# vgl-hub/teloscope

Measured on AMD Instinct MI355X. Metric: Gbases/s scanned (whole node), 3 Gb FASTA TTAGGG w=1000 s=500, higher is better.
Workload: dtype u8; 1 GPU; configs[1]: synthetic 3.00 Gb / 200 contigs, -c TTAGGG -p TTAGGG,TCAGGG,TGAGGG,TTGGGG -x 1 -w 1000 -s 500 -r -g -e -m -i, 124 patterns k=6; bases=3000000000, windows=6000095, matches=91510666, tiles=260970

## Files before the change

teloscope_amd/csrc/capi.cpp:

```cpp
#include <hip/hip_runtime.h>
#include <immintrin.h>

#include <algorithm>
#include <atomic>
#include <thread>
#include <cstdio>
#include <cstddef>
#include <cstdlib>
#include <chrono>
#include <cstring>
#include <limits>
#include <memory>
#include <mutex>
#include <string>
#include <tuple>
#include <vector>

#include <cctype>
#include <pthread.h>
#include <sched.h>
#include <sys/mman.h>

#include "capi_internal.hpp"

// ... 713 lines not shown
    if (!ctx) return TS_ERR_INVALID_ARG;
    DEVICE_TRY(ctx);
    int ok = 0;
    if (ts_k_streams_concurrent(stream_a, stream_b, &ok) != 0) return ctx->fail(TS_ERR_HIP, "stream probe failed");
    return ok;
}

int ts_refresh_env(ts_ctx *ctx) {
    if (!ctx) return TS_ERR_INVALID_ARG;
    std::lock_guard<std::mutex> lk(ctx->api_mtx);
    read_env_knobs(ctx);
    return TS_OK;
}

int ts_takes_text_input(const ts_ctx *ctx, int tips_only) {
    std::string why;
    return ctx && ((tips_only ? ctx->fast_ok : ts_full_scan_supported(ctx, why)) || ctx->generic_ok) ? 1 : 0;
}

int ts_device_input_stats(const ts_ctx *ctx, uint64_t out[4]) {
    if (!ctx || !out) return TS_ERR_INVALID_ARG;
    for (int i = 0; i < 4; ++i) out[i] = ctx->device_input_stats[i].load(std::memory_order_relaxed);
    return TS_OK;
}

int ts_upload_stats(const ts_ctx *ctx, uint64_t out[8]) {
    if (!ctx || !out) return TS_ERR_INVALID_ARG;
    for (int i = 0; i < 8; ++i) out[i] = ctx->upload_stats[i].load(std::memory_order_relaxed);
    return TS_OK;
}

ts_batch *ts_batch_create(ts_ctx *ctx, const uint64_t *seg_lens, const uint64_t *abs_pos,
                          size_t n_segs, int tips_only, uint64_t match_capacity) {
    if (!ctx) return nullptr;
    if (n_segs && !seg_lens) { ctx->fail(TS_ERR_INVALID_ARG, "ts_batch_create: null seg_lens"); return nullptr; }
    std::string why;
    if (tips_only ? !ctx->fast_ok : !ts_full_scan_supported(ctx, why)) {
        ctx->fail(TS_ERR_UNSUPPORTED, "unsupported parameter set: " + (tips_only ? ctx->why_not : why));
        return nullptr;
    }

    ts_batch *b = new ts_batch();
    b->ctx = ctx;
    b->tips = tips_only != 0;
    uint32_t wpt = 1;
    if (!plan_geometry(ctx, b->tips, b->kp, wpt, why)) {
        ctx->fail(TS_ERR_UNSUPPORTED, "unsupported parameter set: " + why);
        delete b;
        return nullptr;
    }
    b->wpt = wpt;
    if (getenv("TS_TIMING"))
        fprintf(stderr, "ts_batch_create: %s scan, k=%u (%s pair table), %u x %u waves per CU, %u chunks and %u windows per tile, LDS %d B per workgroup "
                        "(match queue %u, record stage %u, %u accumulator copies)\n", b->tips ? "tips-only" : "window", ctx->k,
                ctx->pair_byte_table ? "byte" : "2-bit",
                b->kp.wgs_per_cu, b->kp.waves_per_wg, b->kp.nch, wpt, ts_k_lds_bytes(&b->kp), (unsigned)TS_LIST, b->kp.stage_cap, b->kp.acc_copies);
    const uint64_t tile_bases = (uint64_t)wpt * b->kp.s;
    const uint32_t tl = ctx->params.terminal_limit;

    uint64_t off = 0, wins = 0;
    b->segs.resize(n_segs);
    for (size_t i = 0; i < n_segs; ++i) {
        SegPlan &sp = b->segs[i];
        sp.len = seg_lens[i];
        sp.abs_pos = abs_pos ? abs_pos[i] : 0;
        sp.in_off = off;
        off += (sp.len + 15) & ~15ull;
        sp.first_tile = (uint32_t)b->tiles.size();
        if (b->tips) {
            const uint32_t twice = 2u * tl;
            if (sp.len > twice) {
                add_region_tiles(b, sp, (uint32_t)i, 0, tl, tile_bases, 1, false);
                add_region_tiles(b, sp, (uint32_t)i, sp.len - tl, tl, tile_bases, 1, false);
            } else if (sp.len > 0) {
                add_region_tiles(b, sp, (uint32_t)i, 0, sp.len, tile_bases, 1, false);
            }
        } else {
            sp.win_base = wins;
            sp.n_windows = ceil_div(sp.len, ctx->params.step);
            wins += sp.n_windows;
            if (sp.len > 0) add_region_tiles(b, sp, (uint32_t)i, 0, sp.len, tile_bases, wpt, true);
        }
        sp.n_tiles = (uint32_t)b->tiles.size() - sp.first_tile;
        b->total_bases += sp.len;
    }
    b->input_bytes = off + TS_IN_PAD;
    b->n_windows = wins;
    b->match_cap_request = match_capacity;
    if (b->tiles.size() >= 0x7FFFFFFFull) {
        ctx->fail(TS_ERR_UNSUPPORTED, "too many tiles in one batch");
        delete b;
        return nullptr;
    }
    b->lds_bytes = (uint32_t)ts_k_lds_bytes(&b->kp);
    b->kp.rec16 = (b->kp.stage_u16 && ctx->knobs.rec16) ? 1u : 0u;
    set_range(b, 0, b->tiles.size());
    return b;
}

void ts_batch_destroy(ts_batch *b) {
    if (!b) return;
    ts_ctx *c = b->ctx;
    if (c->device != kNoDevice) {
        DeviceGuard g(c->device);
        for (DevBuf *d : {&b->d_in, &b->d_tiles, &b->d_windows, &b->d_matches, &b->d_tile_off, &b->d_stats, &b->d_fill, &b->d_tickets,
                          &b->d_segtab, &b->d_dense, &b->d_dense_base, &b->d_scan_tmp, &b->d_readtab, &b->d_shard_segs,
                          &b->d_shard_bounds, &b->d_shard_tmp, &b->d_shard_cand, &b->d_vis, &b->d_chain, &b->d_zone})
            c->pool.give(std::move(*d));
        for (hipEvent_t e : b->evs)
// ... 806 lines not shown
```

teloscope_amd/csrc/kernels.hip:

```cpp
#include <hip/hip_runtime.h>
#include <stdint.h>

#include <type_traits>

#include "ts_device.h"
#include "ts_internal.h"

#define set_prio(p) __builtin_amdgcn_s_setprio(p)
constexpr int kPrioPass = 3;
constexpr int kPrioAppend = 2;
constexpr int kPrioWindows = 2;

namespace {

typedef unsigned long long u64;
#define LDS __attribute__((address_space(3)))
typedef uint32_t u32x2 __attribute__((ext_vector_type(2)));
typedef LDS unsigned char lds_u8;
typedef LDS uint16_t lds_u16;
typedef LDS uint32_t lds_u32;

__device__ __forceinline__ lds_u16 *lds_at16(uint32_t addr) { return (lds_u16 *)(uintptr_t)addr; }
__device__ __forceinline__ lds_u8 *lds_at8(uint32_t addr) { return (lds_u8 *)(uintptr_t)addr; }

__host__ __device__ inline uint32_t align16(uint32_t x) { return (x + 15u) & ~15u; }

struct SliceLayout { uint32_t codes, rec, wacc, stage, park, bytes; };

__host__ __device__ inline SliceLayout slice_layout(const TsScanParams &P) {
    SliceLayout s;
    uint32_t o = 0;
    s.codes = o; o += align16((P.nch * 63u + 1u) * 8u);
    s.rec = o; o += (P.windows_on && P.nuc_on) ? align16((P.max_windows + P.halo_blocks) * 16u) : 0u;
    s.wacc = o; o += P.windows_on ? align16((P.max_windows + (P.acc_blocks ? P.halo_blocks : 0u)) * 8u * (P.acc_copies + (P.acc_blocks ? 1u : 0u))) : 0u;
    s.stage = o; o += (P.stage_cap + 64u) * (P.stage_u16 ? 2u : 4u);
    s.park = o; o += 32u;
    s.bytes = o;
    return s;
}

__host__ __device__ inline uint32_t queue_region(const TsScanParams &P) {
    const uint32_t a = TS_LIST * 2u;
    return (P.table_rows * 4u + P.fc_bytes + a - 1u) & ~(a - 1u);
}

__host__ __device__ inline uint32_t lds_total(const TsScanParams &P) {
    return queue_region(P) + P.waves_per_wg * (TS_LIST * 2u + slice_layout(P).bytes);
}

template <bool FC_BYTES, bool PAIR_BYTES, int WAVES_EU, bool EMIT, bool FAST>
__global__ __launch_bounds__(TS_MAX_WG_THREADS, WAVES_EU)
void ts_scan_tiles(const TsScanParams P) {
    const bool st16 = FAST ? true : P.stage_u16 != 0u;
    const bool accb = FAST ? true : P.acc_blocks != 0u;
    extern __shared__ __attribute__((aligned(16))) unsigned char lds_raw[];
    const uint32_t tid = threadIdx.x;
    const uint32_t lane = tid & 63u;
    const uint32_t wave = (uint32_t)__builtin_amdgcn_readfirstlane((int)(tid >> 6));

    const uint32_t table_bytes = P.table_rows * 4u + P.fc_bytes;
    {
        const uint4 *src = (const uint4 *)P.table;
        uint4 *dst = (uint4 *)lds_raw;
        const uint32_t n16 = table_bytes >> 4;
        for (uint32_t i = tid; i < n16; i += blockDim.x) dst[i] = src[i];
    }
    __syncthreads();

    const SliceLayout SL = slice_layout(P);
    lds_u8 *lds = (lds_u8 *)lds_raw;
    uint32_t qbase = queue_region(P) + wave * (TS_LIST * 2u);
    uint32_t qmask = TS_LIST * 2u - 2u;
    asm volatile("" : "+v"(qbase));
    asm volatile("" : "+s"(qmask));
    lds_u8 *slice = lds + queue_region(P) + P.waves_per_wg * (TS_LIST * 2u) + wave * SL.bytes;
    lds_u32 *codes = (lds_u32 *)(slice + SL.codes);
    lds_u32 *rec = (lds_u32 *)(slice + SL.rec);
    lds_u32 *stage = (lds_u32 *)(slice + SL.stage);
    LDS u64 *wacc = (LDS u64 *)(slice + SL.wacc);
    lds_u32 *park = (lds_u32 *)(slice + SL.park);
    const uint32_t acc_rows = P.max_windows + (accb ? P.halo_blocks : 0u);
    const uint32_t acc_off = (lane & (P.acc_copies - 1u)) * acc_rows;

    const uint32_t k = P.k;
    const uint32_t rowbits = 2u * (k + 1u) - 4u;
    const uint32_t kmask = (1u << (2u * k)) - 1u;
    const uint32_t pmask = (1u << (2u * (k + 1u))) - 1u;
    const lds_u32 *fc_table = (const lds_u32 *)(lds + P.table_rows * 4u);
    const lds_u8 *fc_bytes = (const lds_u8 *)fc_table;
    const uint32_t tab_base = (uint32_t)(uintptr_t)lds;
    if (PAIR_BYTES && (tab_base & pmask) != 0u) __builtin_trap();

    const uint32_t total_waves = gridDim.x * P.waves_per_wg;
    const uint32_t gw = blockIdx.x * P.waves_per_wg + wave;
    typedef const TsScanParams __attribute__((address_space(4))) *KernArgs;
    auto tail_params = [&]() -> KernArgs {
        KernArgs q = (KernArgs)__builtin_amdgcn_kernarg_segment_ptr();
        asm volatile("" : "+s"(q));
        return q;
    };
    uint32_t cursor = 0;
    if (EMIT) { park[4] = 0u; park[5] = 0u; }
    const uint32_t nwper = P.halo_blocks + 1u;

    typedef const TsTile __attribute__((address_space(4))) *ConstTiles;
    const ConstTiles const_tiles = (ConstTiles)(uintptr_t)P.tiles;
    uint4 n0 = make_uint4(0, 0, 0, 0), n1 = n0;
// ... 166 lines not shown
                                     "s_and_b64 %[m], %[m], %[canm]\n\t"
                                     "s_bcnt1_i32_b64 %[tmp], %[m]\n\t"
                                     "s_cmp_lg_u64 %[H], 0\n\t"
                                     "s_cselect_b32 %[cc], %[tmp], %[t]"
                                     : [cc] "+s"(ch_cc), [w1] "+s"(ch_w1), [tmp] "=&s"(tmp), [m] "=&s"(m)
                                     : [H] "s"(H), [canm] "s"(canm), [t] "s"(t)
                                     : "scc");
                    }
                }
                ch_last = (uint32_t)__builtin_amdgcn_readlane((int)u, FULL ? 63 : (int)nrow - 1);
            };
            if (!redo) {
                const uint32_t nfull = n & ~63u;
                for (uint32_t i0 = 0; i0 < nfull; i0 += 64u) {
                    const uint32_t o = cursor + base + i0 + ln;
                    const uint32_t r = stage_at(i0 + ln);
                    auto put = [&]() { if (rec16) gstore_lo16(wave_out16 + o, r); else gstore(wave_out + o, r); };
                    if (rec_fit) put();
                    else if (o < cap) put();
                    look(r, 64u, i0, std::true_type{});
                }
                for (uint32_t i0 = nfull; i0 < n; i0 += 64u) {
                    const uint32_t nrow = n - i0 < 64u ? n - i0 : 64u;
                    const uint32_t o = cursor + base + i0 + ln;
                    uint32_t r = 0u;
                    if (ln < nrow) {
                        r = stage_at(i0 + ln);
                        if (o < cap) {
                            if (rec16) gstore_lo16(wave_out16 + o, r);
                            else gstore(wave_out + o, r);
                        }
                    }
                    look(r, nrow, i0, std::false_type{});
                }
            } else {
                for (uint32_t i0 = 0; i0 < n; i0 += 64u) {
                    const uint32_t nrow = n - i0 < 64u ? n - i0 : 64u;
                    const uint32_t o = cursor + base + i0 + ln;
                    uint32_t r = 0u;
                    if (ln < nrow && o < cap)
                        r = rec16 ? (uint32_t)__hip_atomic_load(wave_out16 + o, __ATOMIC_RELAXED, __HIP_MEMORY_SCOPE_AGENT)
                                  : __hip_atomic_load(wave_out + o, __ATOMIC_RELAXED, __HIP_MEMORY_SCOPE_AGENT);
                    look(r, nrow, i0, std::false_type{});
                }
            }
            flushed = done;
            const uint32_t z15 = ch_cc < 0x7FFFu ? ch_cc : 0x7FFFu;
            if (!(ch_w1 & TS_CHAIN_HEADS)) ch_w1 |= z15;
            const u64 voff = vwave + vbase;
            if (ln == 0u) gstore((uint4 *)&Q->tile_chain[4ull * tile], make_uint4((ch_first & 0xFFFFu) | (ch_last << 16), ch_w1 | (z15 << 16), (uint32_t)voff, (uint32_t)(voff >> 32)));
            tile_vis = vout;
            park[4] = vbase + vout;
        };
        if (P.windows_on)
            for (uint32_t it = lane; it < acc_rows * 2u * (P.acc_copies + (accb ? 1u : 0u)); it += 64u) ((lds_u32 *)wacc)[it] = 0u;

        uint32_t qhead = 0, qcount = 0;
        auto drain_queue = [&](const uint32_t threshold) {
            if (qcount >= threshold && qcount > 0u) set_prio(kPrioPass);
            while (qcount >= threshold && qcount > 0u) {
                const uint32_t n = qcount < 64u ? qcount : 64u;
                if (done - flushed + 64u > P.stage_cap) flush_stage();
                const bool live = lane < n;
                const uint32_t xp = live ? (uint32_t)*lds_at16(((qhead + lane * 2u) & qmask) | qbase) : 0u;
                const lds_u32 *cw = codes + __builtin_amdgcn_ubfe(xp, 4, 12);
                const uint32_t kw = __builtin_amdgcn_alignbit(cw[1], cw[0], (xp & 15u) * 2u);
                const uint32_t idx = kw & kmask;
                uint32_t fc;
                if (PAIR_BYTES) fc = __builtin_amdgcn_ubfe((uint32_t)*lds_at8(kw & pmask), 2, 2);
                else if (FC_BYTES) fc = fc_bytes[idx];
                else fc = (fc_table[idx >> 4] >> ((idx & 15u) << 1)) & 3u;
                const uint32_t u = xp - sh;
                uint32_t q = 0u, o = u;
                if (P.windows_on) {
                    uint32_t qs;
                    if (P.div_exact) {
                        q = __umul24(u, P.s_magic22) >> 22; qs = __umul24(q, P.s);
                    } else {
                        q = __umul24(u, P.s_inv) >> 16; qs = __umul24(q, P.s);
                        if (qs > u) { --q; qs -= P.s; }
                    }
                    o = u - qs;
                }
                u64 valid_m = low_bits(n) & ballot64(xp >= sh);
                if (P.straddle_fix) valid_m &= ~ballot64(o + k > P.s);
                const u64 bal = valid_m & ballot64(xp < own_end);
                const bool valid = __builtin_amdgcn_inverse_ballot_w64(valid_m), owned = __builtin_amdgcn_inverse_ballot_w64(bal);
                const uint32_t rank = __builtin_amdgcn_mbcnt_hi((uint32_t)(bal >> 32), __builtin_amdgcn_mbcnt_lo((uint32_t)bal, 0u));
                const uint32_t slot = owned ? (done - flushed) + rank : P.stage_cap + lane;
                const uint32_t record = (u << 2) | fc;
                if (st16) ((lds_u16 *)stage)[slot] = (uint16_t)record; else stage[slot] = record;
                done += (uint32_t)__popcll(bal);
                const u64 can_all = ballot64((fc & 1u) != 0u), fwd_all = ballot64((fc & 2u) != 0u);
                const bool is_can = __builtin_amdgcn_inverse_ballot_w64(can_all), is_fwd = __builtin_amdgcn_inverse_ballot_w64(fwd_all);
                const u64 canm = can_all & bal;
                ccan += (uint32_t)__popcll(canm);
                cfwd += (uint32_t)__popcll(fwd_all & bal);
                const u64 inc = (u64)(is_can ? 1u : 0x10000u) | ((u64)(is_fwd ? 1u : 0x10000u) << 32);
                if (P.windows_on && accb) {
                    if (valid && q < nblk) atomicAdd((unsigned long long *)(wacc + acc_off + q), inc);
                    const u64 over = valid_m & ballot64(o + k > P.s);
                    if (over != 0ull) {
                        if (__builtin_amdgcn_inverse_ballot_w64(over) && q < nblk) atomicAdd((unsigned long long *)(wacc + P.acc_copies * acc_rows + q), inc);
                    }
                } else if (P.windows_on) {
                    for (uint32_t j = 0; j < nwper; ++j) {
                        const uint32_t wi = q - j;
                        const bool in = valid && wi < T.nwin && o + k + j * P.s <= P.w;
                        if (in) atomicAdd((unsigned long long *)(wacc + acc_off + wi), inc);
                    }
                }
                qhead = (qhead + 2u * n) & (TS_LIST * 2u - 1u);
                qcount -= n;
            }
            set_prio(0);
            __builtin_amdgcn_wave_barrier();
        };

        auto scan_chunk = [&](const uint32_t cpos, const uint32_t ch, const uint4 v0, const uint4 v1) -> uint32_t {
            const uint32_t x[8] = {v0.x, v0.y, v0.z, v0.w, v1.x, v1.y, v1.z, v1.w};
            uint32_t t[8], e[8], bad = 0;
#pragma unroll
            for (int i = 0; i < 8; ++i) {
                t[i] = x[i] & 0x06060606u;
                e[i] = __builtin_amdgcn_perm(0xFF47FF54u, 0xFF43FF41u, t[i]);
                bad = __builtin_amdgcn_bitop3_b32(x[i], e[i], bad, 0xBE);
            }
            uint32_t wa = pack16(t), wb = pack16(t + 4);

            const uint32_t pos0 = cpos + lane * 32u;
            uint32_t inv = 0;
            const bool slow = __any((bad & P.fold_mask) != 0u) || (cpos + 2048u > xend);
            if (slow) {
                asm volatile("; non-ACGT bases or segment end in this chunk" ::: "memory");
                uint32_t b4[8];
#pragma unroll
                for (int i = 0; i < 8; ++i) {
                    const uint32_t d = (x[i] & P.fold_mask) ^ e[i];
                    const uint32_t nz = ((((d & 0x7F7F7F7Fu) + 0x7F7F7F7Fu) | d) & 0x80808080u) >> 7;
                    b4[i] = __builtin_amdgcn_udot4(nz, 0x08040201u, 0u, false);
                }
                inv = b4[0] | (b4[1] << 4) | (b4[2] << 8) | (b4[3] << 12) |
                      (b4[4] << 16) | (b4[5] << 20) | (b4[6] << 24) | (b4[7] << 28);
                uint32_t inside = inv;
                if (pos0 < sh) inside &= ~0u << (sh - pos0);
                if (pos0 + 32u > xend) {
                    const uint32_t nv = xend > pos0 ? xend - pos0 : 0u;
                    inside &= ~(~0u << nv);
                    inv |= ~0u << nv;
                }
                if (__any(inside != 0u)) has_invalid = true;
                wa = pack16(t); wb = pack16(t + 4);
            }

            const uint32_t nx = (uint32_t)__builtin_amdgcn_mov_dpp((int)wa, 0x130, 0xf, 0xf, false);

            uint32_t tmp[16], ent[16];
            const uint32_t xa = PAIR_BYTES ? __builtin_amdgcn_alignbit(wb, wa, 16) : 0u;
            const uint32_t xb = PAIR_BYTES ? __builtin_amdgcn_alignbit(nx, wb, 16) : 0u;
#pragma unroll
            for (int j = 0; j < 16; ++j) {
                if (PAIR_BYTES) {
                    tmp[j] = 0;
// ... 45 lines not shown
                    incl = wave_scan_add(nm);
                    total = (uint32_t)__builtin_amdgcn_readlane((int)incl, 63);
                }
                drain_queue(qcount + total > TS_LIST ? 1u : 64u);
                uint32_t o = qhead + 2u * (qcount + incl - nm);
                while (m) {
                    *lds_at16((o & qmask) | qbase) = (uint16_t)(lbase + (uint32_t)__builtin_ctz(m));
                    o += 2u;
                    m &= m - 1u;
                }
                qcount += total;
                __builtin_amdgcn_wave_barrier();
            }
        };
        auto append_pair = [&](const uint32_t mA, const uint32_t cposA, const uint32_t mB, const uint32_t cposB) {
            if (!__any((mA | mB) != 0u)) return;
            set_prio(kPrioAppend);
            const uint32_t nA = __popc(mA), nB = __popc(mB);
            const uint32_t incl = wave_scan_add(nA | (nB << 16));
            const uint32_t tot = (uint32_t)__builtin_amdgcn_readlane((int)incl, 63);
            const uint32_t totA = tot & 0xFFFFu, totB = tot >> 16;
            if (totA + totB + 63u > TS_LIST) {
                asm volatile("; dense pair of chunks" ::: "memory");
                if (totA) append_chunk(mA, cposA, nA, incl & 0xFFFFu, totA);
                if (totB) append_chunk(mB, cposB, nB, incl >> 16, totB);
                set_prio(0);
                return;
            }
            drain_queue(64u);
            set_prio(kPrioAppend);
            uint32_t o = qhead + 2u * (qcount + (incl & 0xFFFFu) - nA), m = mA;
            uint32_t lbase = cposA + lane * 32u;
            while (m) {
                *lds_at16((o & qmask) | qbase) = (uint16_t)(lbase + (uint32_t)__builtin_ctz(m));
                o += 2u;
                m &= m - 1u;
            }
            o = qhead + 2u * (qcount + totA + (incl >> 16) - nB); m = mB;
            lbase = cposB + lane * 32u;
            while (m) {
                *lds_at16((o & qmask) | qbase) = (uint16_t)(lbase + (uint32_t)__builtin_ctz(m));
                o += 2u;
                m &= m - 1u;
            }
            qcount += totA + totB;
            set_prio(0);
            __builtin_amdgcn_wave_barrier();
        };
        {
            const uint32_t last_pos = (uint32_t)__builtin_amdgcn_readfirstlane((int)((nch - 1u) * TS_CHUNK));
            const unsigned char *lsrc = src + lane * 32u;
            uint4 a0 = n0, a1 = n1, b0, b1;
            uint32_t cpos = 0, ch = 0;
            for (uint32_t c = 0; c < nch; c += 2u) {
                const uint32_t p1 = cpos + TS_CHUNK < last_pos ? cpos + TS_CHUNK : last_pos;
                b0 = *(const uint4 *)(lsrc + p1);
                b1 = *(const uint4 *)(lsrc + p1 + 16);
                __builtin_amdgcn_sched_barrier(0);
                const uint32_t mA = scan_chunk(cpos, ch, a0, a1);
                uint32_t mB = 0u;
                const bool pair = c + 1u < nch;
                if (pair) {
                    const uint32_t p2 = cpos + 2u * TS_CHUNK < last_pos ? cpos + 2u * TS_CHUNK : last_pos;
                    a0 = *(const uint4 *)(lsrc + p2);
                    a1 = *(const uint4 *)(lsrc + p2 + 16);
                    __builtin_amdgcn_sched_barrier(0);
                    mB = scan_chunk(cpos + TS_CHUNK, ch + 63u, b0, b1);
                }
                append_pair(mA, cpos, mB, cpos + TS_CHUNK);
                cpos += 2u * TS_CHUNK; ch += 126u;
            }
        }
#define TS_REQUEST_NEXT_TILE()                                                                                                   \
        {                                                                                                                        \
                           \
            __builtin_amdgcn_s_waitcnt(0x0F70);                                                                                  \
            KernArgs Q = tail_params();                                                                                          \
            const bool dyn = Q->dynamic_tiles != 0u;                                                                             \
            tile_next = dyn ? group + Q->ticket_groups * (group_waves + (uint32_t)__builtin_amdgcn_readfirstlane((int)ticket))   \
                            : tile + total_waves;                                                                                \
            if (tile_next < P.ntiles) {                       \
                const unsigned char *ls = P.in + (const_tiles[tile_next].in_off & ~15ull) + lane * 32u;                          \
                n0 = *(const uint4 *)ls; n1 = *(const uint4 *)(ls + 16);                                                         \
                if (dyn && lane == 0) ticket = take_ticket(Q);                         \
            }                                                                                                                    \
        }
        if (!EMIT) TS_REQUEST_NEXT_TILE()
        drain_queue(1u);
        __builtin_amdgcn_wave_barrier();

        set_prio(kPrioWindows);
        if (!EMIT) finish_records();
        if (EMIT) TS_REQUEST_NEXT_TILE()
        if (P.windows_on) {
            auto count_piece = [&](uint32_t xs, uint32_t xe, uint32_t &nL, uint32_t &nH, uint32_t &nG) {
                const uint32_t d0 = xs >> 4, d1 = (xe - 1u) >> 4;
                const uint32_t m0 = ~0u << (2u * (xs & 15u));
                const uint32_t m1 = ~0u >> (2u * (15u - ((xe - 1u) & 15u)));
                auto add2 = [&](uint32_t wA, uint32_t wB) {
                    const uint32_t lo = (wA & 0x55555555u) | ((wB << 1) & 0xAAAAAAAAu);
                    const uint32_t hi = ((wA >> 1) & 0x55555555u) | (wB & 0xAAAAAAAAu);
                    nL += __popc(lo); nH += __popc(hi); nG += __popc(lo & hi);
                };
                uint32_t first = codes[d0] & m0, last = 0u;
                if (d1 == d0) first &= m1; else last = codes[d1] & m1;
                add2(first, last);
                uint32_t d = d0 + 1u;
                for (; d + 2u <= d1; d += 2u) add2(codes[d], codes[d + 1u]);
                if (d < d1) add2(codes[d], 0u);
            };
            auto count_piece_bytes = [&](uint32_t xs, uint32_t xe, uint32_t n[4]) {
                const uint32_t fold = P.fold_mask & 0xFFu;
                for (uint32_t x = xs; x < xe; ++x) {
                    const uint32_t c = (uint32_t)src[x] & fold;
                    n[0] += c == 0x41u; n[1] += c == 0x43u; n[2] += c == 0x47u; n[3] += c == 0x54u;
                }
            };
            const bool by_blocks = P.block_sums != 0u;
            if (P.nuc_on) {
                const uint32_t rows = by_blocks ? T.nwin + P.halo_blocks : T.nwin;
                const uint32_t len = by_blocks ? P.s : P.w;
                for (uint32_t it = lane; it < rows * 4u; it += 64u) rec[it] = 0u;
                uint32_t pshift = 0;
                while (pshift < 2u && (rows << (pshift + 1u)) <= 64u && (len >> (pshift + 1u)) >= 128u) ++pshift;
                const uint32_t piece = (len + (1u << pshift) - 1u) >> pshift;
                __builtin_amdgcn_wave_barrier();
                for (uint32_t it = lane; it < (rows << pshift); it += 64u) {
                    const uint32_t row = it >> pshift, part = it & ((1u << pshift) - 1u);
                    const uint32_t row_end = row * P.s + len < T.nrel ? row * P.s + len : T.nrel;
                    const uint32_t us = row * P.s + part * piece;
                    const uint32_t ue = us + piece < row_end ? us + piece : row_end;
                    if (us >= ue) continue;
                    uint32_t n[4] = {0u, 0u, 0u, 0u};
                    if (has_invalid) {
                        count_piece_bytes(sh + us, sh + ue, n);
                    } else {
                        uint32_t nL = 0, nH = 0, nG = 0;
                        count_piece(sh + us, sh + ue, nL, nH, nG);
                        n[0] = (ue - us) + nG - nL - nH; n[1] = nL - nG; n[2] = nG; n[3] = nH - nG;
                    }
                    LDS uint32_t *r4 = rec + row * 4u;
                    if (pshift == 0u) { r4[0] = n[0]; r4[1] = n[1]; r4[2] = n[2]; r4[3] = n[3]; }
                    else {
#pragma unroll
                        for (int f = 0; f < 4; ++f) (void)__hip_atomic_fetch_add(r4 + f, n[f], __ATOMIC_RELAXED, __HIP_MEMORY_SCOPE_WORKGROUP);
                    }
                }
// ... 92 lines not shown
        __builtin_amdgcn_wave_barrier();
    }
    if (lane == 0) {
        KernArgs Q = tail_params();
        Q->wave_fill[gw] = cursor;
        if (EMIT) Q->wave_fill[total_waves + gw] = park[4];
    }
}

__global__ void ts_segment_summary(const uint32_t *tile_stats, const uint32_t *seg_first_tile,
                                   const uint64_t *seg_nwin, uint32_t nseg, u64 *out) {
    __shared__ u64 part[3][256];
    const uint32_t sidx = blockIdx.x;
    if (sidx >= nseg) return;
    const uint32_t t0 = seg_first_tile[sidx], t1 = seg_first_tile[sidx + 1];
    u64 nm = 0, nc = 0, nf = 0;
    for (uint32_t t = t0 + threadIdx.x; t < t1; t += blockDim.x) {
        const uint4 st = *(const uint4 *)&tile_stats[4ull * t];
        nm += st.x; nc += st.y; nf += st.z;
    }
    part[0][threadIdx.x] = nm; part[1][threadIdx.x] = nc; part[2][threadIdx.x] = nf;
    __syncthreads();
    for (uint32_t o = 128; o >= 1; o >>= 1) {
        if (threadIdx.x < o) {
            part[0][threadIdx.x] += part[0][threadIdx.x + o];
            part[1][threadIdx.x] += part[1][threadIdx.x + o];
            part[2][threadIdx.x] += part[2][threadIdx.x + o];
        }
        __syncthreads();
    }
    if (threadIdx.x == 0) {
        out[4ull * sidx + 0] = seg_nwin[sidx];
        out[4ull * sidx + 1] = part[0][0];
        out[4ull * sidx + 2] = part[1][0];
        out[4ull * sidx + 3] = part[2][0];
    }
}

__global__ void ts_compact_regions(const uint32_t *regions, const uint32_t *wave_fill, const u64 *wave_dense_base,
                                   uint32_t region_cap, uint32_t nwaves, uint32_t *dense, int rec16) {
    const uint32_t w = blockIdx.x;
    if (w >= nwaves) return;
    const uint32_t n = wave_fill[w] < region_cap ? wave_fill[w] : region_cap;
    uint32_t *dst = dense + wave_dense_base[w];
    if (rec16) { const uint16_t *src = (const uint16_t *)regions + (u64)w * region_cap; for (uint32_t i = threadIdx.x; i < n; i += blockDim.x) dst[i] = src[i]; }
    else { const uint32_t *src = regions + (u64)w * region_cap; for (uint32_t i = threadIdx.x; i < n; i += blockDim.x) dst[i] = src[i]; }
}

}

int ts_k_lds_bytes(const TsScanParams *p) { return (int)lds_total(*p); }

namespace {
template <bool EMIT>
const void *scan_variant_e(const TsScanParams *p) {
    const bool two = p->wgs_per_cu > 1u;
    if (p->pair_byte_table && p->fc_byte_table) {
        const bool fast = p->stage_u16 && (!p->windows_on || p->acc_blocks);
        if (fast) return two ? (const void *)ts_scan_tiles<true, true, 6, EMIT, true> : (const void *)ts_scan_tiles<true, true, 4, EMIT, true>;
        return two ? (const void *)ts_scan_tiles<true, true, 6, EMIT, false> : (const void *)ts_scan_tiles<true, true, 4, EMIT, false>;
    }
    if (two) return nullptr;
    if (p->fc_byte_table) return (const void *)ts_scan_tiles<true, false, 4, EMIT, false>;
    return (const void *)ts_scan_tiles<false, false, 4, EMIT, false>;
}
const void *scan_variant(const TsScanParams *p) { return p->emit ? scan_variant_e<true>(p) : scan_variant_e<false>(p); }
}

int ts_k_prepare(uint32_t lds_bytes) {
    const void *fns[] = {(const void *)ts_scan_tiles<true, true, 4, false, false>, (const void *)ts_scan_tiles<true, false, 4, false, false>,
                         (const void *)ts_scan_tiles<false, false, 4, false, false>, (const void *)ts_scan_tiles<true, true, 6, false, false>,
                         (const void *)ts_scan_tiles<true, true, 4, true, false>, (const void *)ts_scan_tiles<true, false, 4, true, false>,
                         (const void *)ts_scan_tiles<false, false, 4, true, false>, (const void *)ts_scan_tiles<true, true, 6, true, false>,
                         (const void *)ts_scan_tiles<true, true, 4, false, true>, (const void *)ts_scan_tiles<true, true, 6, false, true>,
                         (const void *)ts_scan_tiles<true, true, 4, true, true>, (const void *)ts_scan_tiles<true, true, 6, true, true>};
    const int limit = (int)(lds_bytes > 160u * 1024u ? lds_bytes : 160u * 1024u);
    for (const void *fn : fns) {
        int e = (int)hipFuncSetAttribute(fn, hipFuncAttributeMaxDynamicSharedMemorySize, limit);
        if (e) return e;
    }
    return 0;
}

int ts_k_launch_scan(const TsScanParams *p, uint32_t grid, uint32_t lds_bytes, void *stream) {
    const dim3 block(p->waves_per_wg * 64u);
    const void *fn = scan_variant(p);
    if (!fn) return (int)hipErrorInvalidConfiguration;
    void *args[] = {(void *)p};
    return (int)hipLaunchKernel(fn, dim3(grid), block, args, lds_bytes, (hipStream_t)stream);
}

int ts_k_launch_summary(const uint32_t *tile_stats, const uint32_t *seg_first_tile, const uint64_t *seg_nwin,
                        uint32_t nseg, unsigned long long *out, void *stream) {
    if (nseg == 0) return 0;
    hipLaunchKernelGGL(ts_segment_summary, dim3(nseg), dim3(256), 0, (hipStream_t)stream,
                       tile_stats, seg_first_tile, seg_nwin, nseg, out);
    return (int)hipGetLastError();
}

int ts_k_launch_compact(const uint32_t *regions, const uint32_t *wave_fill, const unsigned long long *wave_dense_base,
                        uint32_t region_cap, uint32_t nwaves, uint32_t *dense, int rec16, void *stream) {
    if (nwaves == 0) return 0;
    hipLaunchKernelGGL(ts_compact_regions, dim3(nwaves), dim3(256), 0, (hipStream_t)stream,
                       regions, wave_fill, wave_dense_base, region_cap, nwaves, dense, rec16);
    return (int)hipGetLastError();
}
```

teloscope_amd/csrc/ts_internal.h:

```cpp
#ifndef TS_INTERNAL_H
#define TS_INTERNAL_H

#include <stdint.h>


#define TS_MAX_WG_THREADS 1024
#ifndef TS_LIST
#define TS_LIST         512
#endif
#define TS_CHUNK        2016
#define TS_BLK_COUNTERS 10
#define TS_TICKET_STRIDE 64
#define TS_MAX_TICKET_GROUPS 64
#define TS_IN_PAD       4096

struct TsTile {
    uint64_t in_off;
    uint64_t win_out;
    uint32_t nrel;
    uint32_t nwin;
    uint32_t own_len;
    uint32_t seg;
};

// ... 171 lines not shown
    uint32_t terminal_limit, k, nuc_on, field_bits;
    unsigned char *msg;
    unsigned long long off_segs, off_windows, off_tilevis, off_visible, off_blocks;
    const uint32_t *chain;
    const void *vis_src;
    uint32_t vis_src_wide;
    uint32_t vis_cap;
};

struct TsGenericPatterns {
    const unsigned long long *codes;
    const uint8_t *flags;
    uint32_t nlen;
    uint32_t len[8];
    uint32_t first[9];
};

struct TsWidePatterns {
    const unsigned long long *lo, *hi;
    const uint8_t *flags;
    const uint32_t *len;
    const uint32_t *first;
    uint32_t nlen, npat;
};
#define TS_WIDE_HALO 64

struct TsGenericGeom {
    uint32_t s, w, longest;
    uint32_t nuc_on, fold;
    uint32_t s_magic;
    uint32_t cw, rw;
};

#define TS_GENERAL_TILE 4096
struct TsGeneralTile {
    unsigned long long in_off;
    unsigned long long seg_rel;
    unsigned long long k_p0;
    uint32_t n;
    uint32_t avail;
    uint32_t seg;
    uint32_t r_p0;
};

struct TsLaunchInfo {
    uint32_t grid;
    uint32_t lds_bytes;
};

#ifdef __cplusplus
extern "C++" {
int  ts_k_lds_bytes(const TsScanParams *p);
int  ts_k_prepare(uint32_t lds_bytes);
int  ts_k_launch_scan(const TsScanParams *p, uint32_t grid, uint32_t lds_bytes, void *stream);
int  ts_k_launch_summary(const uint32_t *tile_stats, const uint32_t *seg_first_tile,
                         const uint64_t *seg_nwin, uint32_t nseg, unsigned long long *out, void *stream);
unsigned long long ts_k_general_lds_bytes(const TsGenericPatterns *G, uint32_t *lds_patterns);
int  ts_k_launch_general_fused(const unsigned char *in, const TsGeneralTile *tiles, uint32_t ntiles,
                               const unsigned long long *seg_len, const unsigned long long *seg_win_base, const unsigned long long *seg_nwin,
                               const TsGenericPatterns *G, const TsGenericGeom *Q, int tips, uint32_t slot_cap,
                               uint32_t *tile_stats, uint32_t *records, uint32_t *win_out, uint32_t *overflow, int list, int num_cu, void *stream);
uint32_t ts_k_general_list_max_records(void);
int  ts_k_launch_general_wide(const unsigned char *in, const TsGeneralTile *tiles, uint32_t ntiles,
                              const unsigned long long *seg_len, const unsigned long long *seg_win_base, const unsigned long long *seg_nwin,
                              const TsWidePatterns *W, const TsGenericGeom *Q, int tips, uint32_t slot_cap,
                              uint32_t *tile_stats, uint32_t *records, uint32_t *win_out, uint32_t *overflow, void *stream);
int  ts_k_launch_general_block_inputs(const TsGeneralTile *gtiles, const unsigned long long *tile_off, const uint32_t *dense,
                                      const unsigned long long *seg_base, uint32_t ntiles, TsTile *tiles, uint32_t *tile_stats,
                                      int count_from_offsets, void *stream);
int  ts_k_launch_general_slot_offsets(unsigned long long *tile_off, uint32_t ntiles, uint32_t slot_cap, void *stream);
int  ts_k_launch_general_compact_push(const TsGeneralTile *gtiles, const uint32_t *tile_stats, unsigned long long *tile_off,
                                      const uint32_t *records, uint32_t slot_cap, uint32_t ntiles, const unsigned long long *seg_len,
                                      uint32_t w, uint32_t s, uint32_t spread, int wide, unsigned long long gen_lens,
                                      const uint32_t *wide_len, uint32_t *dense, void *stream);
int  ts_k_launch_general_compact(const uint32_t *tile_stats, const unsigned long long *tile_off, const uint32_t *records,
                                 uint32_t slot_cap, uint32_t ntiles, uint32_t *dense, void *stream);
int  ts_k_launch_predicate(const TsTile *tiles, const unsigned long long *tile_off, const uint32_t *tile_stats,
                           const uint32_t *matches, unsigned long long nrec_limit, const uint32_t *seg_first_tile,
                           const unsigned long long *seg_in_off, const unsigned long long *seg_len,
                           uint32_t nseg, const TsPredParams *Q, unsigned char *pass, uint32_t *long_list,
                           uint32_t *long_count, int all_terminal, const uint32_t *wave_fill, uint32_t region_cap,
                           uint32_t nwaves, uint32_t *overflow, int rec16, void *stream);
int  ts_k_launch_terminal_ends(const TsTile *tiles, const unsigned long long *tile_off, const uint32_t *tile_stats,
                               const uint32_t *matches, unsigned long long nrec_limit, const uint32_t *seg_first_tile,
                               const unsigned long long *seg_in_off, const unsigned long long *seg_len, uint32_t nseg,
                               const TsPredParams *Q, uint32_t *ends, uint32_t *long_list, uint32_t *long_count, int all_terminal,
                               const uint32_t *wave_fill, uint32_t region_cap, uint32_t nwaves, uint32_t *overflow, int rec16,
                               void *stream);
int  ts_k_launch_block_call(const TsBlockCallParams *Q, const TsShardSegIn *segs, uint32_t nseg, uint32_t seg_base,
                            uint32_t ntiles, unsigned long long *bounds, TsShardSeg *seg_out, int with_its,
                            const TsVisibleOut *vis, unsigned long long *sums, const uint32_t *chain, uint32_t *work, void *stream);
int  ts_k_launch_terminal(const TsBlockCallParams *Q, const TsShardSegIn *segs, uint32_t nseg, uint32_t seg_base, uint32_t ntiles,
                          unsigned long long *bounds, TsShardSeg *seg_out, void *stream);
int  ts_k_launch_segment_sums(const TsBlockCallParams *Q, const TsShardSegIn *segs, uint32_t nseg, uint32_t seg_base, uint32_t ntiles,
                              unsigned long long *sums, TsShardSeg *seg_out, int prezeroed, void *stream);
int  ts_k_launch_zero(void *p0, unsigned long long n0, void *p1, unsigned long long n1, void *p2, unsigned long long n2,
                      void *p3, unsigned long long n3, void *stream);
int  ts_k_launch_interstitial(const TsBlockCallParams *Q, const TsShardSegIn *segs, uint32_t nseg, uint32_t seg_base, uint32_t ntiles,
                              const unsigned long long *bounds, TsShardSeg *seg_out, const TsVisibleOut *vis,
                              const uint32_t *chain, uint32_t *work, int prezeroed, void *stream);
int  ts_k_launch_shard_count(const TsShardPackParams *P, const TsShardHeader *H, void *tmp, int with_visible, TsVisibleOut *vis, void *stream);
int  ts_k_launch_shard_visible(const TsShardPackParams *P, const TsShardHeader *H, void *tmp, int prezeroed, void *stream);
void *ts_k_shard_big_counter(void *tmp, uint32_t own_tiles);
int  ts_k_launch_shard_windows(const TsShardPackParams *P, const TsShardHeader *H, void *stream);
int  ts_k_streams_concurrent(void *a, void *b, int *concurrent);
int  ts_k_launch_shard_overflow(const TsShardPackParams *P, void *stream);
// ... 56 lines not shown
```

Baseline: 4181 Gbases/s.

## Add specialized fast-window scan variants with an all-interior match pass shortcut

```diff
diff --git a/teloscope_amd/csrc/capi.cpp b/teloscope_amd/csrc/capi.cpp
--- a/teloscope_amd/csrc/capi.cpp
+++ b/teloscope_amd/csrc/capi.cpp
@@ -789,9 +789,9 @@
     b->wpt = wpt;
     if (getenv("TS_TIMING"))
         fprintf(stderr, "ts_batch_create: %s scan, k=%u (%s pair table), %u x %u waves per CU, %u chunks and %u windows per tile, LDS %d B per workgroup "
-                        "(match queue %u, record stage %u, %u accumulator copies)\n", b->tips ? "tips-only" : "window", ctx->k,
+                        "(match queue %u, record stage %u, %u accumulator copies), scan build: %s\n", b->tips ? "tips-only" : "window", ctx->k,
                 ctx->pair_byte_table ? "byte" : "2-bit",
-                b->kp.wgs_per_cu, b->kp.waves_per_wg, b->kp.nch, wpt, ts_k_lds_bytes(&b->kp), (unsigned)TS_LIST, b->kp.stage_cap, b->kp.acc_copies);
+                b->kp.wgs_per_cu, b->kp.waves_per_wg, b->kp.nch, wpt, ts_k_lds_bytes(&b->kp), (unsigned)TS_LIST, b->kp.stage_cap, b->kp.acc_copies, ts_k_scan_build(&b->kp));
     const uint64_t tile_bases = (uint64_t)wpt * b->kp.s;
     const uint32_t tl = ctx->params.terminal_limit;
 
diff --git a/teloscope_amd/csrc/kernels.hip b/teloscope_amd/csrc/kernels.hip
--- a/teloscope_amd/csrc/kernels.hip
+++ b/teloscope_amd/csrc/kernels.hip
@@ -48,11 +48,15 @@
     return queue_region(P) + P.waves_per_wg * (TS_LIST * 2u + slice_layout(P).bytes);
 }
 
-template <bool FC_BYTES, bool PAIR_BYTES, int WAVES_EU, bool EMIT, bool FAST>
+enum : int { TS_FAST_NONE = 0, TS_FAST_STAGE = 1, TS_FAST_WINDOWS = 2, TS_FAST_TIPS = 3 };
+template <bool FC_BYTES, bool PAIR_BYTES, int WAVES_EU, bool EMIT, int FAST>
 __global__ __launch_bounds__(TS_MAX_WG_THREADS, WAVES_EU)
 void ts_scan_tiles(const TsScanParams P) {
     const bool st16 = FAST ? true : P.stage_u16 != 0u;
     const bool accb = FAST ? true : P.acc_blocks != 0u;
+    const bool win_on = FAST == TS_FAST_WINDOWS ? true : FAST == TS_FAST_TIPS ? false : P.windows_on != 0u;
+    const bool div_ex = FAST == TS_FAST_WINDOWS ? true : P.div_exact != 0u;
+    const bool straddle = FAST >= TS_FAST_WINDOWS ? false : P.straddle_fix != 0u;
     extern __shared__ __attribute__((aligned(16))) unsigned char lds_raw[];
     const uint32_t tid = threadIdx.x;
     const uint32_t lane = tid & 63u;
@@ -325,7 +329,7 @@
             tile_vis = vout;
             park[4] = vbase + vout;
         };
-        if (P.windows_on)
+        if (win_on)
             for (uint32_t it = lane; it < acc_rows * 2u * (P.acc_copies + (accb ? 1u : 0u)); it += 64u) ((lds_u32 *)wacc)[it] = 0u;
 
         uint32_t qhead = 0, qcount = 0;
@@ -345,9 +349,9 @@
                 else fc = (fc_table[idx >> 4] >> ((idx & 15u) << 1)) & 3u;
                 const uint32_t u = xp - sh;
                 uint32_t q = 0u, o = u;
-                if (P.windows_on) {
+                if (win_on) {
                     uint32_t qs;
-                    if (P.div_exact) {
+                    if (div_ex) {
                         q = __umul24(u, P.s_magic22) >> 22; qs = __umul24(q, P.s);
                     } else {
                         q = __umul24(u, P.s_inv) >> 16; qs = __umul24(q, P.s);
@@ -355,33 +359,59 @@
                     }
                     o = u - qs;
                 }
+                const uint32_t record = (u << 2) | fc;
+                const u64 can_all = ballot64((fc & 1u) != 0u), fwd_all = ballot64((fc & 2u) != 0u);
+                const bool is_can = __builtin_amdgcn_inverse_ballot_w64(can_all), is_fwd = __builtin_amdgcn_inverse_ballot_w64(fwd_all);
+                const u64 inc = (u64)(is_can ? 1u : 0x10000u) | ((u64)(is_fwd ? 1u : 0x10000u) << 32);
+                const bool interior = n == 64u && !straddle
+                                      && (uint32_t)__builtin_amdgcn_readfirstlane((int)xp) >= sh
+                                      && (uint32_t)__builtin_amdgcn_readlane((int)xp, 63) < own_end;
+                if (interior) {
+                    const uint32_t slot = (done - flushed) + lane;
+                    if (st16) ((lds_u16 *)stage)[slot] = (uint16_t)record; else stage[slot] = record;
+                    done += 64u;
+                    ccan += (uint32_t)__popcll(can_all);
+                    cfwd += (uint32_t)__popcll(fwd_all);
+                    if (win_on && accb) {
+                        atomicAdd((unsigned long long *)(wacc + acc_off + q), inc);
+                        const u64 over = ballot64(o + k > P.s);
+                        if (over != 0ull) {
+                            if (__builtin_amdgcn_inverse_ballot_w64(over)) {
+                                atomicAdd((unsigned long long *)(wacc + P.acc_copies * acc_rows + q), inc);
+                                asm volatile("; run-over row of an all-owned pass");
+                            }
+                        }
+                    } else if (win_on) {
+                        for (uint32_t j = 0; j < nwper; ++j) {
+                            const uint32_t wi = q - j;
+                            if (wi < T.nwin && o + k + j * P.s <= P.w) atomicAdd((unsigned long long *)(wacc + acc_off + wi), inc);
+                        }
+                    }
+                } else {
                 u64 valid_m = low_bits(n) & ballot64(xp >= sh);
-                if (P.straddle_fix) valid_m &= ~ballot64(o + k > P.s);
+                if (straddle) valid_m &= ~ballot64(o + k > P.s);
                 const u64 bal = valid_m & ballot64(xp < own_end);
                 const bool valid = __builtin_amdgcn_inverse_ballot_w64(valid_m), owned = __builtin_amdgcn_inverse_ballot_w64(bal);
                 const uint32_t rank = __builtin_amdgcn_mbcnt_hi((uint32_t)(bal >> 32), __builtin_amdgcn_mbcnt_lo((uint32_t)bal, 0u));
                 const uint32_t slot = owned ? (done - flushed) + rank : P.stage_cap + lane;
-                const uint32_t record = (u << 2) | fc;
                 if (st16) ((lds_u16 *)stage)[slot] = (uint16_t)record; else stage[slot] = record;
                 done += (uint32_t)__popcll(bal);
-                const u64 can_all = ballot64((fc & 1u) != 0u), fwd_all = ballot64((fc & 2u) != 0u);
-                const bool is_can = __builtin_amdgcn_inverse_ballot_w64(can_all), is_fwd = __builtin_amdgcn_inverse_ballot_w64(fwd_all);
                 const u64 canm = can_all & bal;
                 ccan += (uint32_t)__popcll(canm);
                 cfwd += (uint32_t)__popcll(fwd_all & bal);
-                const u64 inc = (u64)(is_can ? 1u : 0x10000u) | ((u64)(is_fwd ? 1u : 0x10000u) << 32);
-                if (P.windows_on && accb) {
+                if (win_on && accb) {
                     if (valid && q < nblk) atomicAdd((unsigned long long *)(wacc + acc_off + q), inc);
                     const u64 over = valid_m & ballot64(o + k > P.s);
                     if (over != 0ull) {
                         if (__builtin_amdgcn_inverse_ballot_w64(over) && q < nblk) atomicAdd((unsigned long long *)(wacc + P.acc_copies * acc_rows + q), inc);
                     }
-                } else if (P.windows_on) {
+                } else if (win_on) {
                     for (uint32_t j = 0; j < nwper; ++j) {
                         const uint32_t wi = q - j;
                         const bool in = valid && wi < T.nwin && o + k + j * P.s <= P.w;
                         if (in) atomicAdd((unsigned long long *)(wacc + acc_off + wi), inc);
                     }
+                }
                 }
                 qhead = (qhead + 2u * n) & (TS_LIST * 2u - 1u);
                 qcount -= n;
@@ -533,23 +563,22 @@
             const unsigned char *lsrc = src + lane * 32u;
             uint4 a0 = n0, a1 = n1, b0, b1;
             uint32_t cpos = 0, ch = 0;
-            for (uint32_t c = 0; c < nch; c += 2u) {
-                const uint32_t p1 = cpos + TS_CHUNK < last_pos ? cpos + TS_CHUNK : last_pos;
-                b0 = *(const uint4 *)(lsrc + p1);
-                b1 = *(const uint4 *)(lsrc + p1 + 16);
+            for (uint32_t c = 0; c + 1u < nch; c += 2u) {
+                b0 = *(const uint4 *)(lsrc + cpos + TS_CHUNK);
+                b1 = *(const uint4 *)(lsrc + cpos + TS_CHUNK + 16);
                 __builtin_amdgcn_sched_barrier(0);
                 const uint32_t mA = scan_chunk(cpos, ch, a0, a1);
-                uint32_t mB = 0u;
-                const bool pair = c + 1u < nch;
-                if (pair) {
-                    const uint32_t p2 = cpos + 2u * TS_CHUNK < last_pos ? cpos + 2u * TS_CHUNK : last_pos;
-                    a0 = *(const uint4 *)(lsrc + p2);
-                    a1 = *(const uint4 *)(lsrc + p2 + 16);
-                    __builtin_amdgcn_sched_barrier(0);
-                    mB = scan_chunk(cpos + TS_CHUNK, ch + 63u, b0, b1);
-                }
+                const uint32_t p2 = cpos + 2u * TS_CHUNK < last_pos ? cpos + 2u * TS_CHUNK : last_pos;
+                a0 = *(const uint4 *)(lsrc + p2);
+                a1 = *(const uint4 *)(lsrc + p2 + 16);
+                __builtin_amdgcn_sched_barrier(0);
+                const uint32_t mB = scan_chunk(cpos + TS_CHUNK, ch + 63u, b0, b1);
                 append_pair(mA, cpos, mB, cpos + TS_CHUNK);
                 cpos += 2u * TS_CHUNK; ch += 126u;
+            }
+            if (nch & 1u) {
+                const uint32_t mA = scan_chunk(cpos, ch, a0, a1);
+                append_pair(mA, cpos, 0u, cpos + TS_CHUNK);
             }
         }
 #define TS_REQUEST_NEXT_TILE()                                                                                                   \
@@ -573,7 +602,7 @@
         set_prio(kPrioWindows);
         if (!EMIT) finish_records();
         if (EMIT) TS_REQUEST_NEXT_TILE()
-        if (P.windows_on) {
+        if (win_on) {
             auto count_piece = [&](uint32_t xs, uint32_t xe, uint32_t &nL, uint32_t &nH, uint32_t &nG) {
                 const uint32_t d0 = xs >> 4, d1 = (xe - 1u) >> 4;
                 const uint32_t m0 = ~0u << (2u * (xs & 15u));
@@ -772,28 +801,42 @@
 int ts_k_lds_bytes(const TsScanParams *p) { return (int)lds_total(*p); }
 
 namespace {
+int scan_fast_kind(const TsScanParams *p) {
+    if (!(p->pair_byte_table && p->fc_byte_table)) return TS_FAST_NONE;
+    if (!(p->stage_u16 && (!p->windows_on || p->acc_blocks))) return TS_FAST_NONE;
+    if (p->windows_on && p->acc_blocks && p->div_exact && !p->straddle_fix) return TS_FAST_WINDOWS;
+    if (!p->windows_on && !p->straddle_fix && p->wgs_per_cu <= 1u) return TS_FAST_TIPS;
+    return TS_FAST_STAGE;
+}
 template <bool EMIT>
 const void *scan_variant_e(const TsScanParams *p) {
     const bool two = p->wgs_per_cu > 1u;
     if (p->pair_byte_table && p->fc_byte_table) {
-        const bool fast = p->stage_u16 && (!p->windows_on || p->acc_blocks);
-        if (fast) return two ? (const void *)ts_scan_tiles<true, true, 6, EMIT, true> : (const void *)ts_scan_tiles<true, true, 4, EMIT, true>;
-        return two ? (const void *)ts_scan_tiles<true, true, 6, EMIT, false> : (const void *)ts_scan_tiles<true, true, 4, EMIT, false>;
+        switch (scan_fast_kind(p)) {
+        case TS_FAST_WINDOWS: return two ? (const void *)ts_scan_tiles<true, true, 6, EMIT, TS_FAST_WINDOWS> : (const void *)ts_scan_tiles<true, true, 4, EMIT, TS_FAST_WINDOWS>;
+        case TS_FAST_TIPS: return (const void *)ts_scan_tiles<true, true, 4, EMIT, TS_FAST_TIPS>;
+        case TS_FAST_STAGE: return two ? (const void *)ts_scan_tiles<true, true, 6, EMIT, TS_FAST_STAGE> : (const void *)ts_scan_tiles<true, true, 4, EMIT, TS_FAST_STAGE>;
+        default: break;
+        }
+        return two ? (const void *)ts_scan_tiles<true, true, 6, EMIT, TS_FAST_NONE> : (const void *)ts_scan_tiles<true, true, 4, EMIT, TS_FAST_NONE>;
     }
     if (two) return nullptr;
-    if (p->fc_byte_table) return (const void *)ts_scan_tiles<true, false, 4, EMIT, false>;
-    return (const void *)ts_scan_tiles<false, false, 4, EMIT, false>;
+    if (p->fc_byte_table) return (const void *)ts_scan_tiles<true, false, 4, EMIT, TS_FAST_NONE>;
+    return (const void *)ts_scan_tiles<false, false, 4, EMIT, TS_FAST_NONE>;
 }
 const void *scan_variant(const TsScanParams *p) { return p->emit ? scan_variant_e<true>(p) : scan_variant_e<false>(p); }
 }
 
 int ts_k_prepare(uint32_t lds_bytes) {
-    const void *fns[] = {(const void *)ts_scan_tiles<true, true, 4, false, false>, (const void *)ts_scan_tiles<true, false, 4, false, false>,
-                         (const void *)ts_scan_tiles<false, false, 4, false, false>, (const void *)ts_scan_tiles<true, true, 6, false, false>,
-                         (const void *)ts_scan_tiles<true, true, 4, true, false>, (const void *)ts_scan_tiles<true, false, 4, true, false>,
-                         (const void *)ts_scan_tiles<false, false, 4, true, false>, (const void *)ts_scan_tiles<true, true, 6, true, false>,
-                         (const void *)ts_scan_tiles<true, true, 4, false, true>, (const void *)ts_scan_tiles<true, true, 6, false, true>,
-                         (const void *)ts_scan_tiles<true, true, 4, true, true>, (const void *)ts_scan_tiles<true, true, 6, true, true>};
+    const void *fns[] = {(const void *)ts_scan_tiles<true, true, 4, false, TS_FAST_NONE>, (const void *)ts_scan_tiles<true, false, 4, false, TS_FAST_NONE>,
+                         (const void *)ts_scan_tiles<false, false, 4, false, TS_FAST_NONE>, (const void *)ts_scan_tiles<true, true, 6, false, TS_FAST_NONE>,
+                         (const void *)ts_scan_tiles<true, true, 4, true, TS_FAST_NONE>, (const void *)ts_scan_tiles<true, false, 4, true, TS_FAST_NONE>,
+                         (const void *)ts_scan_tiles<false, false, 4, true, TS_FAST_NONE>, (const void *)ts_scan_tiles<true, true, 6, true, TS_FAST_NONE>,
+                         (const void *)ts_scan_tiles<true, true, 4, false, TS_FAST_STAGE>, (const void *)ts_scan_tiles<true, true, 6, false, TS_FAST_STAGE>,
+                         (const void *)ts_scan_tiles<true, true, 4, true, TS_FAST_STAGE>, (const void *)ts_scan_tiles<true, true, 6, true, TS_FAST_STAGE>,
+                         (const void *)ts_scan_tiles<true, true, 4, false, TS_FAST_WINDOWS>, (const void *)ts_scan_tiles<true, true, 6, false, TS_FAST_WINDOWS>,
+                         (const void *)ts_scan_tiles<true, true, 4, true, TS_FAST_WINDOWS>, (const void *)ts_scan_tiles<true, true, 6, true, TS_FAST_WINDOWS>,
+                         (const void *)ts_scan_tiles<true, true, 4, false, TS_FAST_TIPS>, (const void *)ts_scan_tiles<true, true, 4, true, TS_FAST_TIPS>};
     const int limit = (int)(lds_bytes > 160u * 1024u ? lds_bytes : 160u * 1024u);
     for (const void *fn : fns) {
         int e = (int)hipFuncSetAttribute(fn, hipFuncAttributeMaxDynamicSharedMemorySize, limit);
@@ -802,6 +845,11 @@
     return 0;
 }
 
+const char *ts_k_scan_build(const TsScanParams *p) {
+    static const char *const names[] = {"general", "fast stage", "fast windows", "fast tips"};
+    return names[scan_fast_kind(p)];
+}
+
 int ts_k_launch_scan(const TsScanParams *p, uint32_t grid, uint32_t lds_bytes, void *stream) {
     const dim3 block(p->waves_per_wg * 64u);
     const void *fn = scan_variant(p);
diff --git a/teloscope_amd/csrc/ts_internal.h b/teloscope_amd/csrc/ts_internal.h
--- a/teloscope_amd/csrc/ts_internal.h
+++ b/teloscope_amd/csrc/ts_internal.h
@@ -247,6 +247,7 @@
 extern "C++" {
 int  ts_k_lds_bytes(const TsScanParams *p);
 int  ts_k_prepare(uint32_t lds_bytes);
+const char *ts_k_scan_build(const TsScanParams *p);
 int  ts_k_launch_scan(const TsScanParams *p, uint32_t grid, uint32_t lds_bytes, void *stream);
 int  ts_k_launch_summary(const uint32_t *tile_stats, const uint32_t *seg_first_tile,
                          const uint64_t *seg_nwin, uint32_t nseg, unsigned long long *out, void *stream);
```

Result: no change. 4201 Gbases/s, median of 6 (+0.5%).
